# slowkow/scde

Hardware: AMD Instinct MI355X
Metric: genes/sec for scde.expression.difference (400-pt grid, 100 randomizations) (higher is better)
Workload: dtype f64; 1 GPU; config3: synthetic 20000 genes x 1000 cells (500/500), 401-pt grid, 100 bootstraps, n.cores=1 seeding; genes_total=20000, genes_per_gpu=20000, cells=1000, grid=401, n_randomizations=100, parallelism=gene-shard x1 (strong)

## Files before the change

### scde_amd/csrc/kernels.hip

```cpp
#include <hip/hip_runtime.h>
#include <algorithm>
#include <cmath>
#include <cstdint>
#include <utility>

#include "device_math.h"
#include "kernels.h"
#include "wave_ops.h"

namespace scde {

__global__ __launch_bounds__(256) void k_cell_prep(const double* __restrict__ models, int ncells, int G, int GS,
                                                   const double* __restrict__ mag, int localtheta,
                                                   int squarelogit, double* __restrict__ mu,
                                                   double* __restrict__ lcfp, double* __restrict__ lcfpr,
                                                   double* __restrict__ theta, double* __restrict__ cellscal,
                                                   double* __restrict__ pq, double* __restrict__ cfpo) {
  const int c = blockIdx.x;
  auto M = [&](int col) { return models[(long long)c + (long long)ncells * col]; };
  const double concb = M(0), conca = M(1), failr = M(2), corrb = M(3), corra = M(4), corrt = M(5);
  const double ltb = M(6), ltt = M(7), ltm = M(8), lts = M(9), ltr = M(10), conca2 = M(11);
  double lmax = -INFINITY;
  for (int k = threadIdx.x; k < G; k += blockDim.x) {
    const double m = mag[k];
// ... 307 lines not shown
  if (phase == 1) {
    c = blockIdx.x * 4 + wid;
    if (c >= a.ncells) return;
    const long long o1 = a.ucl_off[c + 1];
    long long zc = -1;
    for (long long i0 = a.ucl_off[c]; i0 < o1; i0 += 64) {
      const long long i = i0 + lane;
      const unsigned long long m = __ballot(i < o1 && a.ucl[i] == 0);
      if (m) {
        zc = i0 + __ffsll((long long)m) - 1;
        break;
      }
    }
    if (lane == 0) a.zcol[c] = zc >= 0 ? (int)zc + a.col_base : -1;
    if (zc < 0) {
      if (lane == 0) a.base_col[c] = -1;
      return;
    }
    col = zc;
  } else {
    col = (long long)blockIdx.x * 4 + wid;
    if (a.slow_only) {
      for (long long b0 = col * 64; b0 < a.ncols; b0 += (long long)gridDim.x * 4 * 64) {
        const long long ci = b0 + lane;
        unsigned long long m = __ballot(ci < a.ncols && !(a.colc[ci * kColc] > 0.0));
        while (m) {
          const long long cs = b0 + __ffsll((long long)m) - 1;
          m &= m - 1;
          int lo = 0, hi = a.ncells;
          while (hi - lo > 1) {
            const int mid = (lo + hi) >> 1;
            if (a.ucl_off[mid] <= cs) lo = mid; else hi = mid;
          }
          if (phase == 2 && cs == tab_zcol(a, lo)) continue;
          const long long co = (long long)lo * a.GS;
          const int bc = (phase == 2) ? tab_base_col(a, lo) : -1;
          const double* base = (bc >= 0 && a.D) ? a.D + (long long)bc * a.GS : nullptr;
          tables_column<CT>(a, cs, lo, phase, a.mu + co, (CT && a.pq) ? a.pq + 4 * co : nullptr, a.lcfpr + co,
                            a.lcfp + co, nullptr, nullptr, a.theta + co, base, vrow + (long long)wid * a.GS, etab,
                            lt, lane, a.GS);
        }
      }
      return;
    }
    if (phase == 2 && col == a.ncols) {
      for (int k = lane; k < a.GS; k += 64)
        if (a.D) a.D[col * a.GS + k] = 0.0;
      if (a.U && lane < kStretchSlots) a.U[col * kStretchSlots + lane] = 0.0;
      if (a.UQ && lane < kQTiles) a.UQ[col * kQTiles + lane] = 0u;
      return;
    }
    if (col >= a.ncols) return;
    int lo = 0, hi = a.ncells;
    while (hi - lo > 1) {
      const int mid = (lo + hi) >> 1;
      if (a.ucl_off[mid] <= col) lo = mid; else hi = mid;
    }
    c = lo;
    if (phase == 2 && col == tab_zcol(a, c)) return;
  }
  const long long co = (long long)c * a.GS;
  const int bc = (phase == 2) ? tab_base_col(a, c) : -1;
  const double* base = (bc >= 0 && a.D) ? a.D + (long long)bc * a.GS : nullptr;
  tables_column<CT>(a, col, c, phase, a.mu + co, (CT && a.pq) ? a.pq + 4 * co : nullptr, a.lcfpr + co,
                    a.lcfp + co, nullptr, nullptr, a.theta + co, base, vrow + (long long)wid * a.GS, etab, lt, lane,
                    a.GS);
}

constexpr int kTabStagedG = 448;
constexpr int kTabWaves = 8;
template <bool CT>
__global__ __launch_bounds__(64 * kTabWaves) __attribute__((amdgpu_waves_per_eu(SCDE_TAB_WPE))) void k_tables_cell(TablesArgs a) {
  extern __shared__ double dyn[];
  __shared__ double etab[64];
  __shared__ unsigned suqb[kQTiles];
  __shared__ double ltab[3][97];
  const int lane = threadIdx.x & 63, wid = threadIdx.x >> 6;
  const int GS = a.GS, G = a.G;
  tables_tabs(etab, ltab);
  if (a.gate && *a.gate == 0) return;
  const int4 task = a.tasks[blockIdx.x];
  const int c = task.x;
  const int phase = a.phase;
  if (c < 0) {
    if (wid == 0) {
      for (int k = lane; k < GS; k += 64)
        if (a.D) a.D[a.ncols * GS + k] = 0.0;
      if (a.U && lane < kStretchSlots) a.U[a.ncols * kStretchSlots + lane] = 0.0;
      if (a.UQ && lane < kQTiles) a.UQ[a.ncols * kQTiles + lane] = 0u;
    }
    return;
  }
  const bool haveP = CT && a.pq;
  double* smu = dyn + kTabWaves * G;
  double* sP = smu + G;
  double* slr = sP + 4 * G;
  double* slc = slr + G;
  double* sth = slc + G;
  double* sbase = sth + G;
  const long long co = (long long)c * GS;
  const int bc = (phase == 2) ? tab_base_col(a, c) : -1;
  if (bc >= 0 && a.UQ && threadIdx.x < kQTiles) suqb[threadIdx.x] = a.UQ[(long long)bc * kQTiles + threadIdx.x];
  for (int k = threadIdx.x; k < G; k += 64 * kTabWaves) {
    smu[k] = a.mu[co + k];
    slr[k] = a.lcfpr[co + k];
    slc[k] = exp(a.lcfp[co + k]);
    sth[k] = a.theta[co + k];
    if (haveP) {
      const double* P = a.pq + 4 * co;
      sP[k] = P[k];
      sP[G + k] = P[GS + k];
      sP[2 * G + k] = P[2 * GS + k];
      sP[3 * G + k] = P[3 * GS + k];
    }
    if (bc >= 0) sbase[k] = a.D[(long long)bc * GS + k];
  }
  __syncthreads();
  const LogTab lt{ltab[0], ltab[1], ltab[2]};
  const int zc = (phase == 2) ? tab_zcol(a, c) : -1;
  for (int col = task.y + wid; col < task.z; col += kTabWaves) {
    if (col == zc) continue;
    tables_column<CT>(a, col, c, phase, smu, haveP ? sP : nullptr, slr, nullptr, slc, (bc >= 0) ? suqb : nullptr, sth,
                      (bc >= 0) ? sbase : nullptr, dyn + wid * G, etab, lt, lane, G);
  }
}

constexpr int kTabChunks = kTabStagedG / 64;

constexpr int kRS = kTabStagedG;
enum { kRowMu = 0, kRowLP = 1, kRowLQ = 2, kRowLcfpr = 3, kRowCfp = 4, kRowLcfp = 5, kRowBase = 6, kTabRegRows = 7 };

enum { kBoundNone = 0, kBoundTiles = 1, kBoundStretch = 2 };
__device__ __forceinline__ void tab_store(double* p, double v, int nt) {
  if (nt)
    __builtin_nontemporal_store(v, p);
  else
    *p = v;
}
typedef double tab_v2d __attribute__((ext_vector_type(2)));
__device__ __forceinline__ void tab_store2(double* p, double a, double b, int nt) {
  tab_v2d v;
  v.x = a;
  v.y = b;
  if (nt)
    __builtin_nontemporal_store(v, reinterpret_cast<tab_v2d*>(p));
  else
    *reinterpret_cast<tab_v2d*>(p) = v;
}

template <int BM, int GC>
__device__ __forceinline__ void tables_column_reg(const TablesArgs& a, long long col, int c, int phase,
                                                  const double* __restrict__ sm, bool have_base,
                                                  const unsigned* __restrict__ uqb, const double* etab,
                                                  const LogTab& lt, int lane, double theta, const double* cc,
                                                  double x, double maxcfp, int bc_u) {
  const int G = GC ? GC : a.G;
  if (!(cc[0] > 0.0)) return;
  const double fp = cc[7];
  const double lpo = cc[8], lqo = cc[9];
  const double po = theta / (theta + x);
  if (SCDE_KT_DIAG & 32) {
    if (po == 12345.0) a.has_clamp[col] = 1;
    return;
  }
  const double* sl = sm + lane;
  double v[kTabChunks];
  double lmax = -INFINITY;
#pragma unroll
  for (int j = 0; j < kTabChunks; ++j) {
    v[j] = -INFINITY;
    if (64 * j < G) {
      const int k = lane + 64 * j;
      const bool in = k < G;
      const bool last = (k == G - 1);
      double lpr = sl[kRowLP * kRS + 64 * j], lqr = sl[kRowLQ * kRS + 64 * j];
      const double muv = sl[kRowMu * kRS + 64 * j], mnext = sl[kRowMu * kRS + 64 * j + 1];
      const bool over = in && ((!last && x > muv && x < mnext) || (last && x > muv));
      if (__builtin_amdgcn_ballot_w64(over)) {
        lpr = over ? lpo : lpr;
        lqr = over ? lqo : lqr;
      }
      double nb = (x == 0.0) ? theta * lpr : fma(x, lqr, fma(theta, lpr, cc[10]));
      nb += sl[kRowLcfpr * kRS + 64 * j];
      v[j] = in ? nb : -INFINITY;
      lmax = gt_max(lmax, v[j]);
    }
  }
  if (SCDE_KT_DIAG & 16) {
    if (lmax == 12345.0) a.has_clamp[col] = 1;
    return;
  }
  double maxp = wave_allreduce<true>(lmax);
  if (maxp < (maxcfp + fp)) maxp = maxcfp + fp;
  const double d0 = fp - maxp;
  const double E = exp_tab(fmax(d0, -746.0), etab);
  double ls = 0.0;
#pragma unroll
  for (int j = 0; j < kTabChunks; ++j) {
    if (64 * j < G) {
      const int k = lane + 64 * j;
      const bool in = k < G;
      v[j] -= maxp;
      double e = sl[kRowCfp * kRS + 64 * j] * E;
      if (!(SCDE_KT_DIAG & 2) && __builtin_amdgcn_ballot_w64(in && v[j] > -60.0)) e += exp_tab(fmax(v[j], -746.0), etab);
      ls += in ? e : 0.0;
    }
  }
  const double s = wave_allreduce<false>(ls);
  const double lsum = log_tab(s, lt);
  const bool want_maxi = a.maxi != nullptr;
  double bv = -INFINITY;
  int bi = 0x7fffffff;
  bool clamp = false, nanq = false;
  double* out = a.T ? a.T + col * a.GS : nullptr;
  double* dout = (phase && a.D) ? a.D + col * a.GS : nullptr;
  const double minlp = a.minlogprob;
  unsigned uqv = 0;
#pragma unroll
  for (int j = 0; j < kTabChunks; ++j) {
    if (64 * j < G) {
      const int k = lane + 64 * j;
      const bool in = k < G;
      const double t1 = v[j], t2 = sl[kRowLcfp * kRS + 64 * j] + d0;
      const double hi = gt_max(t2, t1), lo = (t1 > t2) ? t2 : t1;
      const bool tiny = !(hi >= -665.0);
      const bool mixed = !tiny && !(hi - lo > 37.5);
      double r = hi - lsum;
      if (__builtin_amdgcn_ballot_w64(in && (tiny || mixed))) {
        double e = fma(sl[kRowCfp * kRS + 64 * j], E, exp_tab(fmax(t1, -746.0), etab));
        if (__builtin_amdgcn_ballot_w64(in && tiny)) {
          const double et = exp_tab(fmax((sl[kRowLcfp * kRS + 64 * j] + fp) - maxp, -746.0), etab) +
                            exp_tab(fmax(t1, -746.0), etab);
          e = tiny ? et : e;
        }
        const double rm = (SCDE_KT_DIAG & 4) ? e - lsum : log_tab(tiny ? e / s : e, lt) - (tiny ? 0.0 : lsum);
        r = (tiny || mixed) ? rm : r;
      }
      if (want_maxi && r > bv && in) {
        bv = r;
        bi = k;
      }
      const bool cl = r < minlp;
      r = cl ? minlp : r;
      clamp = clamp || (cl && in);
      nanq = nanq || (in && r != r);
      if (!(SCDE_KT_DIAG & 8)) {
        if (out) tab_store(out + k, in ? r : 0.0, a.nt_rows);
        if (dout) tab_store(dout + k, in ? (have_base ? r - sl[kRowBase * kRS + 64 * j] : r) : 0.0, a.nt_rows);
      } else if (r == 12345.0) {
        dout[k] = r;
      }
      r = in ? r : -INFINITY;
      if (BM == kBoundTiles && !(SCDE_KT_DIAG & 64)) {
        int u = row16_max_i32((int)ceil(fmax(r * 256.0, -0x1p29)));
        const auto sw = __builtin_amdgcn_permlane16_swap((unsigned)u, (unsigned)u, false, false);
        u = max((int)sw[0], (int)sw[1]);
        const int g = __builtin_amdgcn_ds_bpermute(((lane - 2 * j) & 1) << 7, u);
        uqv = ((lane >> 1) == j) ? (unsigned)g : uqv;
      }
      if (BM == kBoundStretch) {
        const float mf = wave_maxf((float)r);
        if (lane == 0) {
          const double m = (double)mf + 0x1p-23 * fabs((double)mf);
          a.U[col * kStretchSlots + j] = (bc_u >= 0) ? m - a.U[(long long)bc_u * kStretchSlots + j] : m;
        }
      }
    }
  }
  if (BM == kBoundTiles) {
    if (__ballot(nanq) && lane == 0) *a.nanflag = 1;
    if (lane < kQTiles) {
      int u = (int)uqv;
      if (kBTile * lane >= G)
        u = 0;
      else if (bc_u >= 0)
        u -= unpacku(uqb[lane]);
      a.UQ[col * kQTiles + lane] = packu(u);
    }
  }
  if (dout)
    for (int k = 64 * ((G + 63) / 64) + lane; k < a.GS; k += 64) dout[k] = 0.0;
  if (want_maxi) {
#pragma unroll
    for (int m = 32; m >= 1; m >>= 1) {
      const double ov = __shfl_xor(bv, m, 64);
      const int oi = __shfl_xor(bi, m, 64);
      if (ov > bv || (ov == bv && oi < bi)) {
        bv = ov;
        bi = oi;
      }
    }
    if (lane == 0) a.maxi[col] = (bi == 0x7fffffff) ? 0 : bi;
  }
  const unsigned long long anyc = __ballot(clamp);
  if (lane == 0) a.has_clamp[col] = anyc ? 1 : 0;
}

#ifndef SCDE_LPC_DIAG
#define SCDE_LPC_DIAG 0
#endif
#ifndef LPC_U12
#define LPC_U12 4
#endif
#ifndef LPC_U3
#define LPC_U3 8
#endif
constexpr int kLpcWaves = 4;
constexpr int kLpcFlush = 8;
constexpr int kLpcTS = kLpcFlush + 1;
constexpr int kLpcQB = 0;
constexpr int kLpcLC = 2 * kTabStagedG;
constexpr int kLpcBase = 4 * kTabStagedG;
constexpr int kLpcR = 5 * kTabStagedG;
constexpr int kLpcMu = kLpcR;
constexpr int kLpcPart = kLpcR + kTabStagedG;
constexpr int kLpcRsz = kLpcWaves * 64 * kLpcTS;
constexpr int kLpcLds0 = kLpcR + kLpcRsz;
constexpr int kLpcLds = kLpcLds0 > kTabRegRows * kRS ? kLpcLds0 : kTabRegRows * kRS;
static_assert(kLpcRsz >= kTabStagedG + kLpcWaves * 64, "mu and the partials fit region R");
static_assert(kLpcWaves * 64 * 3 <= kLpcBase, "the combine's arrays overlay the staged rows");
static_assert(kTabTaskCols <= 64, "k_tables_lpc maps one lane to each column of a task: wider tasks would lose columns");

template <int BM>
__global__ __launch_bounds__(64 * kLpcWaves) void k_tables_lpc(TablesArgs a) {
  __shared__ __attribute__((aligned(16))) double lds[kLpcLds];
  __shared__ double etab[64];
  __shared__ unsigned suqb[kQTiles];
  __shared__ unsigned spart2[kLpcWaves][2][64];
  double(*spart)[64] = reinterpret_cast<double(*)[64]>(lds + kLpcPart);
  __shared__ int sfb[64];
  __shared__ int nfb;
  const int lane = threadIdx.x & 63;
  const int w = __builtin_amdgcn_readfirstlane(threadIdx.x >> 6);
  const int GS = a.GS, G = a.G;
  if (threadIdx.x < 64) etab[threadIdx.x] = kExp2Frac64[threadIdx.x];
  if (a.gate && *a.gate == 0) return;
  const int4 task = a.tasks[blockIdx.x];
  const int c = task.x;
  if (c < 0) {
    if (w == 0) {
      for (int k = lane; k < GS; k += 64)
        if (a.D) a.D[a.ncols * GS + k] = 0.0;
      if (a.U && lane < kStretchSlots) a.U[a.ncols * kStretchSlots + lane] = 0.0;
      if (a.UQ && lane < kQTiles) a.UQ[a.ncols * kQTiles + lane] = 0u;
    }
    return;
  }
  const int phase = a.phase;
  const long long co = (long long)c * GS;
  const int bc = (phase == 2) ? tab_base_col(a, c) : -1;
  if (bc >= 0 && a.UQ && threadIdx.x < kQTiles) suqb[threadIdx.x] = a.UQ[(long long)bc * kQTiles + threadIdx.x];
  if (threadIdx.x == 0) nfb = 0;
  const double theta = a.theta[co];
  const double* P = a.pq + 4 * co;
  int lean = theta > 0.0 && theta <= DBL_MAX;
  for (int k = threadIdx.x; k < kTabStagedG; k += 64 * kLpcWaves) {
    const bool in = k < G;
    double lq = 0.0, B = 0.0, lc = -INFINITY, cf = 0.0, base = 0.0, mu = 0.0;
    if (in) {
      mu = a.mu[co + k];
      const double lp = P[2 * GS + k], lr = a.lcfpr[co + k];
      lq = P[3 * GS + k];
      lc = a.lcfp[co + k];
      cf = a.cfp ? a.cfp[co + k] : exp(lc);
      B = fma(theta, lp, lr);
      if (bc >= 0) base = a.D[(long long)bc * GS + k];
      const bool ok = (k == G - 1 || mu <= a.mu[co + k + 1]) && lp <= DBL_MAX && lq <= DBL_MAX && lr <= DBL_MAX &&
                      lc <= DBL_MAX && cf <= DBL_MAX && cf == cf;
      lean &= ok ? 1 : 0;
    }
    lds[kLpcQB + 2 * k] = lq;
    lds[kLpcQB + 2 * k + 1] = B;
    lds[kLpcLC + 2 * k] = lc;
    lds[kLpcLC + 2 * k + 1] = cf;
    lds[kLpcBase + k] = base;
    lds[kLpcMu + k] = mu;
  }
  lean = __syncthreads_and(lean);
  const LogTab lt{kLogInvC, kLogCHi, kLogCLo};
  const int zc = (phase == 2) ? tab_zcol(a, c) : -1;
  const double maxcfp = a.cellscal[2 * c];
  const double minlp = a.minlogprob;
  const int col = task.y + lane;
  const bool mine = col < task.z && col != zc;
  double x = 1.0, c10 = 0.0, fp = 0.0, lpo = -1.0, lqo = -1.0;
  bool ok = false;
  if (mine) {
    const double* cc = a.colc + (long long)col * kColc;
    const double xx = (double)a.ucl[col], n = cc[0], cten = cc[10];
    if (lean && xx > 0.0 && n > 0.0 && cten >= -DBL_MAX && cten <= DBL_MAX) {
      ok = true;
      x = xx;
      c10 = cten;
      fp = cc[7];
      lpo = cc[8];
      lqo = cc[9];
    }
  }
  int ks = -1;
  double nb0o = 0.0;
  {
    int lo = 0, hi = G;
    while (lo < hi) {
      const int mid = (lo + hi) >> 1;
      if (lds[kLpcMu + mid] < x) lo = mid + 1; else hi = mid;
    }
    if (lo >= 1 && (lo == G || x < lds[kLpcMu + lo])) {
      ks = lo - 1;
      nb0o = fma(x, lqo, fma(theta, lpo, a.lcfpr[co + ks]));
    }
  }
  const int Gr = (G + kLpcFlush - 1) / kLpcFlush * kLpcFlush;
  const int per = max(64, (Gr / kLpcFlush + kLpcWaves - 1) / kLpcWaves * kLpcFlush);
  const int k0 = min(Gr, w * per), k1 = min(G, k0 + per), k1r = min(Gr, k0 + per);
  const double2* QB = reinterpret_cast<const double2*>(lds + kLpcQB);
  const double2* LC = reinterpret_cast<const double2*>(lds + kLpcLC);
  double m = -INFINITY;
#pragma unroll LPC_U12
  for (int k = k0; k < k1; ++k) {
    const double2 qb = QB[k];
    double nb = fma(x, qb.x, qb.y);
    nb = (k == ks) ? nb0o : nb;
    nb += c10;
    m = fmax(m, nb);
  }
  spart[w][lane] = m;
  __syncthreads();
  m = fmax(fmax(fmax(spart[0][lane], spart[1][lane]), spart[2][lane]), spart[3][lane]);
  double maxp = m;
  if (maxp < (maxcfp + fp)) maxp = maxcfp + fp;
  ok = ok && maxp > -INFINITY && maxp < INFINITY;
  if (!ok) maxp = 0.0;
  const double d0 = fp - maxp;
  const double E = exp_tab(fmax(d0, -746.0), etab);
  double ls = 0.0;
#pragma unroll LPC_U12
  for (int k = k0; k < k1; ++k) {
    const double2 qb = QB[k];
    const double cf = LC[k].y;
    const double t1 = (fma(x, qb.x, qb.y) + c10) - maxp;
    double e = cf * E;
    if (!(SCDE_LPC_DIAG & 2)) e += exp_tab(fmax(t1, -746.0), etab);
    ls += e;
  }
  if (ks >= k0 && ks < k1) {
    const double cf = LC[ks].y, tp = (fma(x, QB[ks].x, QB[ks].y) + c10) - maxp, to = (nb0o + c10) - maxp;
    ls += (cf * E + exp_tab(fmax(to, -746.0), etab)) - (cf * E + exp_tab(fmax(tp, -746.0), etab));
  }
  __syncthreads();
  spart[w][lane] = ls;
  __syncthreads();
  const double sq = ((spart[0][lane] + spart[1][lane]) + spart[2][lane]) + spart[3][lane];
  const double lsum = log_tab(sq, lt);
  __syncthreads();
  const bool want_maxi = a.maxi != nullptr;
  double bv = -INFINITY;
  int bi = 0x7fffffff;
  unsigned long long clampm = 0;
  const unsigned long long okm = __builtin_amdgcn_ballot_w64(ok);
  double* tw = lds + kLpcR + w * 64 * kLpcTS;
  double* const T = a.T;
  double* const D = (phase && a.D) ? a.D : nullptr;
  const long long cbase = task.y;
  constexpr int BSZ = (BM == kBoundStretch) ? 64 : kBTile;
  auto bound_form = [&](double mx) -> unsigned {
    if (BM == kBoundTiles) return (unsigned)(int)ceil(fmax(mx * 256.0, -0x1p29));
    return __float_as_uint((float)mx);
  };
  auto bound_max = [&](unsigned p, unsigned q) -> unsigned {
    if (BM == kBoundTiles) return (unsigned)max((int)p, (int)q);
    return __float_as_uint(fmaxf(__uint_as_float(p), __uint_as_float(q)));
  };
  auto put_bound = [&](int seg, unsigned form) {
    if (!ok) return;
    if (BM == kBoundTiles) {
      int u = (int)form;
      if (bc >= 0) u -= unpacku(suqb[seg]);
      a.UQ[(long long)col * kQTiles + seg] = packu(u);
    } else if (BM == kBoundStretch) {
      const float mf = __uint_as_float(form);
      const double mm = (double)mf + 0x1p-23 * fabs((double)mf);
      a.U[(long long)col * kStretchSlots + seg] = (bc >= 0) ? mm - a.U[(long long)bc * kStretchSlots + seg] : mm;
    }
  };
  double bt = -INFINITY;
  for (int f0 = k0; f0 < k1r; f0 += kLpcFlush) {
#pragma unroll LPC_U3
    for (int kk = 0; kk < kLpcFlush; ++kk) {
      const int k = f0 + kk;
      double r = 0.0;
      if (k < k1) {
        const double2 qb = QB[k], lcf = LC[k];
        double nb = fma(x, qb.x, qb.y);
        nb = (k == ks) ? nb0o : nb;
        const double t1 = (nb + c10) - maxp, t2 = lcf.x + d0;
        const double hi = fmax(t2, t1);
        const bool tiny = !(hi >= -665.0);
        const bool tm = tiny || !(fabs(t1 - t2) > 37.5);
        r = hi - lsum;
        if (!(SCDE_LPC_DIAG & 4) && __builtin_amdgcn_ballot_w64(ok && tm)) {
          double e = fma(lcf.y, E, exp_tab(fmax(t1, -746.0), etab));
          if (__builtin_amdgcn_ballot_w64(ok && tiny)) {
            const double et = exp_tab(fmax((lcf.x + fp) - maxp, -746.0), etab) + exp_tab(fmax(t1, -746.0), etab);
            e = tiny ? et / sq : e;
          }
          const double rm = log_tab(e, lt) - (tiny ? 0.0 : lsum);
          r = tm ? rm : r;
        }
        if (want_maxi) {
          const bool better = r > bv;
          bv = better ? r : bv;
          bi = better ? k : bi;
        }
        clampm |= __builtin_amdgcn_ballot_w64(r < minlp);
        r = fmax(r, minlp);
        if (BM != kBoundNone) {
          bt = fmax(bt, r);
          if ((k % BSZ) == BSZ - 1 || k == k1 - 1) {
            const int seg = k / BSZ;
            const bool head = seg * BSZ < k0, tail = (k % BSZ) != BSZ - 1 && k != G - 1;
            if (!head && !tail)
              put_bound(seg, bound_form(bt));
            else
              spart2[w][tail ? 1 : 0][lane] = bound_form(bt);
            bt = -INFINITY;
          }
        }
      }
      tw[lane * kLpcTS + kk] = r;
    }
#pragma unroll
    for (int i = 0; i < ((SCDE_LPC_DIAG & 1) ? 0 : 4); ++i) {
      const int cc_ = i * 16 + (lane >> 2), kp = (lane & 3) * 2;
      if ((okm >> cc_) & 1ull) {
        const double r0 = tw[cc_ * kLpcTS + kp], r1 = tw[cc_ * kLpcTS + kp + 1];
        const long long off = (cbase + cc_) * GS + f0 + kp;
        if (T) tab_store2(T + off, r0, r1, a.nt_rows);
        if (D) {
          const double2 bb = *reinterpret_cast<const double2*>(lds + kLpcBase + f0 + kp);
          tab_store2(D + off, r0 - bb.x, r1 - bb.y, a.nt_rows);
        }
      }
    }
  }
  const int GP = (SCDE_LPC_DIAG & 8) ? GS : min(GS, (G + 63) / 64 * 64);
  for (int f0 = Gr + kLpcFlush * w; f0 < GP; f0 += kLpcFlush * kLpcWaves) {
#pragma unroll
    for (int i = 0; i < 4; ++i) {
      const int cc_ = i * 16 + (lane >> 2), kp = (lane & 3) * 2;
      if ((okm >> cc_) & 1ull) {
        const long long off = (cbase + cc_) * GS + f0 + kp;
        const double z = ((SCDE_LPC_DIAG & 8) && f0 >= (G + 63) / 64 * 64) ? __builtin_nan("") : 0.0;
        if (T) tab_store2(T + off, z, z, a.nt_rows);
        if (D) tab_store2(D + off, z, z, a.nt_rows);
      }
    }
  }
  __syncthreads();
  double(*sclamp)[64] = reinterpret_cast<double(*)[64]>(lds);
  double(*sbv)[64] = reinterpret_cast<double(*)[64]>(lds + kLpcWaves * 64);
  int(*sbi)[64] = reinterpret_cast<int(*)[64]>(lds + 2 * kLpcWaves * 64);
  sclamp[w][lane] = ((clampm >> lane) & 1ull) ? 1.0 : 0.0;
  sbi[w][lane] = bi;
  sbv[w][lane] = bv;
  __syncthreads();
  if (w == 0 && ok) {
    a.has_clamp[col] = (sclamp[0][lane] + sclamp[1][lane] + sclamp[2][lane] + sclamp[3][lane] > 0.0) ? 1 : 0;
    if (want_maxi) {
      double b = sbv[0][lane];
      int bix = sbi[0][lane];
      for (int v = 1; v < kLpcWaves; ++v)
        if (sbv[v][lane] > b) {
          b = sbv[v][lane];
          bix = sbi[v][lane];
        }
      a.maxi[col] = (bix == 0x7fffffff) ? 0 : bix;
    }
  }
  if (BM != kBoundNone && w > 0 && (k0 % BSZ) != 0 && k0 < G)
    put_bound(k0 / BSZ, bound_max(spart2[w - 1][1][lane], spart2[w][0][lane]));
  if (BM == kBoundTiles && w == kLpcWaves - 1)
    for (int t = (G + kBTile - 1) / kBTile; t < kQTiles; ++t)
      if (ok) a.UQ[(long long)col * kQTiles + t] = packu(0);
  if (w == 0 && mine && !ok) sfb[atomicAdd(&nfb, 1)] = col;
  __syncthreads();
  const int nf = nfb;
  if (nf == 0) return;
  double* sm = lds;
  for (int k = threadIdx.x; k < kRS; k += 64 * kLpcWaves) {
    const bool in = k < G;
    sm[kRowMu * kRS + k] = in ? a.mu[co + k] : 0.0;
    sm[kRowLP * kRS + k] = in ? P[2 * GS + k] : 0.0;
    sm[kRowLQ * kRS + k] = in ? P[3 * GS + k] : 0.0;
    sm[kRowLcfpr * kRS + k] = in ? a.lcfpr[co + k] : 0.0;
    const double lc = in ? a.lcfp[co + k] : -INFINITY;
    sm[kRowCfp * kRS + k] = in ? (a.cfp ? a.cfp[co + k] : exp(lc)) : 0.0;
    sm[kRowLcfp * kRS + k] = lc;
    sm[kRowBase * kRS + k] = (in && bc >= 0) ? a.D[(long long)bc * GS + k] : 0.0;
  }
  __syncthreads();
  for (int i = w; i < nf; i += kLpcWaves) {
    const int fc = __builtin_amdgcn_readfirstlane(sfb[i]);
    tables_column_reg<BM, 0>(a, fc, c, phase, sm, bc >= 0, suqb, etab, lt, lane, theta, a.colc + (long long)fc * kColc,
                             (double)a.ucl[fc], maxcfp, bc);
  }
}

__global__ void k_base_cols(const int* __restrict__ ucl, const long long* __restrict__ ucl_off, int ncells,
                            const unsigned char* __restrict__ has_clamp, int use_baseline,
                            int* __restrict__ base_col) {
  const int c = blockIdx.x * blockDim.x + threadIdx.x;
  if (c >= ncells) return;
  int bc = -1;
  if (use_baseline) {
    for (long long i = ucl_off[c]; i < ucl_off[c + 1]; ++i) {
      if (ucl[i] == 0) {
        if (!has_clamp[i]) bc = (int)i;
        break;
      }
    }
  }
  base_col[c] = bc;
}

__global__ __launch_bounds__(256) void k_delta(const double* __restrict__ T, const long long* __restrict__ ucl_off,
                                              int ncells, long long ncols, const int* __restrict__ base_col, int G,
                                              int GS, double* __restrict__ D) {
  const int lane = threadIdx.x & 63;
  const long long col = (long long)blockIdx.x * 4 + (threadIdx.x >> 6);
  if (col > ncols) return;
  if (col == ncols) {
    for (int k = lane; k < GS; k += 64) D[col * GS + k] = 0.0;
    return;
  }
  int lo = 0, hi = ncells;
  while (hi - lo > 1) {
    const int mid = (lo + hi) >> 1;
    if (ucl_off[mid] <= col) lo = mid; else hi = mid;
  }
  const int bc = base_col[lo];
  for (int k = lane; k < GS; k += 64) {
    const double t = (k < G) ? T[col * GS + k] : 0.0;
    D[col * GS + k] = (bc >= 0 && k < G) ? t - T[(long long)bc * GS + k] : t;
  }
}

constexpr int kZWaves = 16;
__global__ __launch_bounds__(64 * kZWaves) void k_baseline_z(const double* __restrict__ T, int G, int GS,
                                                            const int* __restrict__ base_col, int ncells,
                                                            const double* __restrict__ Wt, int Bp,
                                                            double* __restrict__ Z, int gsets, int gsplit) {
  __shared__ double part[kZWaves][4][64];
  const int lane = threadIdx.x & 63, wid = threadIdx.x >> 6;
  const int b0 = blockIdx.x * 4, k = blockIdx.y * 64 + lane, set = blockIdx.z;
  const double* W = Wt + (long long)set * ncells * Bp + b0;
  const bool g2 = gsets > 0 && set >= gsets;
  const int clo = g2 ? gsplit : 0, chi = (gsets > 0 && !g2) ? gsplit : ncells;
  double z[4] = {0.0, 0.0, 0.0, 0.0};
  if (k < G) {
    for (int c = clo + wid; c < chi; c += kZWaves) {
      const int bc = base_col[c];
      if (bc < 0) continue;
      const double t = T[(long long)bc * GS + k];
      const double* w = W + (long long)c * Bp;
#pragma unroll
      for (int r = 0; r < 4; ++r) z[r] = fma(w[r], t, z[r]);
    }
  }
#pragma unroll
  for (int r = 0; r < 4; ++r) part[wid][r][lane] = z[r];
  __syncthreads();
  if (wid < 4 && k < GS) {
    double s = part[0][wid][lane];
#pragma unroll
    for (int w = 1; w < kZWaves; ++w) s += part[w][wid][lane];
    Z[((long long)set * Bp + b0 + wid) * GS + k] = s;
  }
}

__global__ __launch_bounds__(256) void k_stretch_zu(const double* __restrict__ U, const int* __restrict__ base_col,
                                                    int ncells, const double* __restrict__ Wt, int Bp,
                                                    double* __restrict__ ZU, int gsets, int gsplit) {
  __shared__ double part[256][kStretchSlots + 1];
  const int b = blockIdx.x, set = blockIdx.y, t = threadIdx.x;
  const double* W = Wt + (long long)set * ncells * Bp + b;
  const bool g2 = gsets > 0 && set >= gsets;
  const int clo = g2 ? gsplit : 0, chi = (gsets > 0 && !g2) ? gsplit : ncells;
  double z[kStretchSlots];
#pragma unroll
  for (int j = 0; j < kStretchSlots; ++j) z[j] = 0.0;
  for (int c = clo + t; c < chi; c += 256) {
    const int bc = base_col[c];
    if (bc < 0) continue;
    const double w = W[(long long)c * Bp];
    const double* u = U + (long long)bc * kStretchSlots;
#pragma unroll
    for (int j = 0; j < kStretchSlots; ++j) z[j] = fma(w, u[j], z[j]);
  }
#pragma unroll
  for (int j = 0; j < kStretchSlots; ++j) part[t][j] = z[j];
  __syncthreads();
  for (int h = 128; h >= 1; h >>= 1) {
    if (t < h)
#pragma unroll
      for (int j = 0; j < kStretchSlots; ++j) part[t][j] += part[t + h][j];
    __syncthreads();
  }
  if (t < kStretchSlots) ZU[((long long)set * Bp + b) * kStretchSlots + t] = part[0][t];
}

template <int BC, bool MAX>
__device__ __forceinline__ double wave_reduce_scatter_v(double (&v)[BC], int lane) {
  static_assert(BC == 4 || BC == 8 || BC == 16, "BC must be 4, 8 or 16");
#pragma unroll
  for (int j = 0; j < BC / 2; ++j) {
    swap32(v[j], v[j + BC / 2]);
    v[j] = red_op<MAX>(v[j], v[j + BC / 2]);
  }
#pragma unroll
  for (int j = 0; j < BC / 4; ++j) {
    swap16(v[j], v[j + BC / 4]);
    v[j] = red_op<MAX>(v[j], v[j + BC / 4]);
  }
  if constexpr (BC >= 8) {
    const bool up = (lane & 8) != 0;
#pragma unroll
    for (int j = 0; j < BC / 8; ++j) {
      const double lo = v[j], hi = v[j + BC / 8];
      v[j] = red_op<MAX>(up ? hi : lo, dpp_d<kDppMirror>(up ? lo : hi));
    }
  }
  if constexpr (BC >= 16) {
    const bool up = (lane & 4) != 0;
    const double lo = v[0], hi = v[1];
    v[0] = red_op<MAX>(up ? hi : lo, dpp_d<kDppHalfMirror>(up ? lo : hi));
  }
  double x = v[0];
  if constexpr (BC <= 4) x = red_op<MAX>(x, dpp_d<kDppMirror>(x));
  if constexpr (BC <= 8) x = red_op<MAX>(x, dpp_d<kDppHalfMirror>(x));
  x = red_op<MAX>(x, dpp_d<kDppXor2>(x));
  x = red_op<MAX>(x, dpp_d<kDppXor1>(x));
  return x;
}

template <int BC, bool MAX, int NB>
__device__ __forceinline__ void wave_partials(const double (&x)[NB], int I0, bool live, double* red, int lane,
                                              int wid) {
  constexpr int L2 = (BC == 16) ? 4 : (BC == 8) ? 3 : (BC == 4) ? 2 : (BC == 2) ? 1 : 0;
  double t[BC];
#pragma unroll
  for (int i = 0; i < BC; ++i) t[i] = x[I0 + i];
  const double r = wave_reduce_scatter_v<BC, MAX>(t, lane);
  const int idx = (lane >> (6 - L2)) & (BC - 1);
  if ((lane & ((64 >> L2) - 1)) == 0) red[wid * 32 + I0 + idx] = r;
}

template <bool MAX, int NB>
__device__ __forceinline__ void block_reduce_all(const double (&x)[NB], bool live, double* red, double* fin,
                                                 int lane, int wid, int nw) {
#pragma unroll
  for (int i0 = 0; i0 + 16 <= NB; i0 += 16) wave_partials<16, MAX, NB>(x, i0, live, red, lane, wid);
  if constexpr ((NB % 16) >= 8) wave_partials<8, MAX, NB>(x, NB - (NB % 16), live, red, lane, wid);
  if constexpr ((NB % 8) >= 4) wave_partials<4, MAX, NB>(x, NB - (NB % 8), live, red, lane, wid);
  __syncthreads();
  if ((int)threadIdx.x < NB) {
    double r = red[threadIdx.x];
    for (int w = 1; w < nw; ++w) r = MAX ? gt_max(r, red[w * 32 + threadIdx.x]) : r + red[w * 32 + threadIdx.x];
    fin[threadIdx.x] = r;
  }
  __syncthreads();
}


template <int BC>
__device__ __forceinline__ float wave_max_scatter_f(float (&v)[BC], int lane) {
  static_assert(BC == 4 || BC == 8 || BC == 16, "BC must be 4, 8 or 16");
#pragma unroll
  for (int j = 0; j < BC / 2; ++j) {
    swap32f(v[j], v[j + BC / 2]);
    v[j] = gt_maxf(v[j], v[j + BC / 2]);
  }
#pragma unroll
  for (int j = 0; j < BC / 4; ++j) {
    swap16f(v[j], v[j + BC / 4]);
    v[j] = gt_maxf(v[j], v[j + BC / 4]);
  }
  if constexpr (BC >= 8) {
    const bool up = (lane & 8) != 0;
#pragma unroll
    for (int j = 0; j < BC / 8; ++j) {
      const float lo = v[j], hi = v[j + BC / 8];
      v[j] = gt_maxf(up ? hi : lo, dpp_f<kDppMirror>(up ? lo : hi));
    }
  }
  if constexpr (BC >= 16) {
    const bool up = (lane & 4) != 0;
    const float lo = v[0], hi = v[1];
    v[0] = gt_maxf(up ? hi : lo, dpp_f<kDppHalfMirror>(up ? lo : hi));
  }
  float x = v[0];
  if constexpr (BC <= 4) x = gt_maxf(x, dpp_f<kDppMirror>(x));
  if constexpr (BC <= 8) x = gt_maxf(x, dpp_f<kDppHalfMirror>(x));
  x = gt_maxf(x, dpp_f<kDppXor2>(x));
  x = gt_maxf(x, dpp_f<kDppXor1>(x));
  return x;
}

template <int BC, int NB>
__device__ __forceinline__ void wave_max_partials(const double (&x)[NB], int I0, float* redf, int lane, int wid) {
  constexpr int L2 = (BC == 16) ? 4 : (BC == 8) ? 3 : 2;
  float t[BC];
// ... 1659 lines not shown
```

Baseline: 3.053 million genes/s.

## Compact divergent exp/log lanes into dense wave work lists per flush block

The flush loop now runs in two passes. The first pass computes a cheap approximation for each of the 8 grid points and records a per-lane bitmask of points that need the exact exp/log path. Lanes with any such point are compacted into a per-wave LDS list. The wave then processes 8 lanes x 8 points per iteration, fetching each source lane's parameters with shuffles, so the expensive transcendental path runs with dense lanes instead of mostly idle divergent ones. The exact results go through the tw scratch buffer, which adds LDS traffic, shuffles and a serial loop over the list; this could cost more than it saves when few lanes diverge or when nearly all do.

```diff
diff --git a/scde_amd/csrc/kernels.hip b/scde_amd/csrc/kernels.hip
--- a/scde_amd/csrc/kernels.hip
+++ b/scde_amd/csrc/kernels.hip
@@ -633,9 +633,6 @@
 #ifndef LPC_U12
 #define LPC_U12 4
 #endif
-#ifndef LPC_U3
-#define LPC_U3 8
-#endif
 constexpr int kLpcWaves = 4;
 constexpr int kLpcFlush = 8;
 constexpr int kLpcTS = kLpcFlush + 1;
@@ -661,6 +658,7 @@
   double(*spart)[64] = reinterpret_cast<double(*)[64]>(lds + kLpcPart);
   __shared__ int sfb[64];
   __shared__ int nfb;
+  __shared__ unsigned short slist[kLpcWaves][64];
   const int lane = threadIdx.x & 63;
   const int w = __builtin_amdgcn_readfirstlane(threadIdx.x >> 6);
   const int GS = a.GS, G = a.G;
@@ -815,29 +813,65 @@
     }
   };
   double bt = -INFINITY;
+  unsigned short* const wl = slist[w];
   for (int f0 = k0; f0 < k1r; f0 += kLpcFlush) {
-#pragma unroll LPC_U3
+    double rr[kLpcFlush];
+    unsigned fm = 0;
+#pragma unroll
     for (int kk = 0; kk < kLpcFlush; ++kk) {
       const int k = f0 + kk;
-      double r = 0.0;
+      rr[kk] = 0.0;
       if (k < k1) {
         const double2 qb = QB[k], lcf = LC[k];
         double nb = fma(x, qb.x, qb.y);
         nb = (k == ks) ? nb0o : nb;
         const double t1 = (nb + c10) - maxp, t2 = lcf.x + d0;
         const double hi = fmax(t2, t1);
+        const bool tm = !(hi >= -665.0) || !(fabs(t1 - t2) > 37.5);
+        rr[kk] = hi - lsum;
+        fm |= (ok && tm) ? (1u << kk) : 0u;
+      }
+    }
+    if (!(SCDE_LPC_DIAG & 4) && __builtin_amdgcn_ballot_w64(fm != 0)) {
+      const unsigned long long bal = __builtin_amdgcn_ballot_w64(fm != 0);
+      const int nl = __popcll(bal);
+      if (fm) wl[__builtin_amdgcn_mbcnt_hi((unsigned)(bal >> 32), __builtin_amdgcn_mbcnt_lo((unsigned)bal, 0u))] =
+          (unsigned short)(lane | (fm << 6));
+#pragma unroll 1
+      for (int r0 = 0; r0 < nl; r0 += 8) {
+        const int j = r0 + (lane >> 3);
+        const int ent = j < nl ? (int)wl[j] : lane;
+        const int sl = ent & 63, kp = lane & 7, k = f0 + kp;
+        const bool live = (ent >> (6 + kp)) & 1;
+        const double xs = __shfl(x, sl, 64), c10s = __shfl(c10, sl, 64), maxps = __shfl(maxp, sl, 64);
+        const double fps = __shfl(fp, sl, 64), Es = __shfl(E, sl, 64), lsums = __shfl(lsum, sl, 64);
+        const double nb0s = __shfl(nb0o, sl, 64);
+        const int kss = __shfl(ks, sl, 64);
+        const double2 qb = QB[k], lcf = LC[k];
+        double nb = fma(xs, qb.x, qb.y);
+        nb = (k == kss) ? nb0s : nb;
+        const double d0s = fps - maxps;
+        const double t1 = (nb + c10s) - maxps, t2 = lcf.x + d0s;
+        const double hi = fmax(t2, t1);
         const bool tiny = !(hi >= -665.0);
-        const bool tm = tiny || !(fabs(t1 - t2) > 37.5);
-        r = hi - lsum;
-        if (!(SCDE_LPC_DIAG & 4) && __builtin_amdgcn_ballot_w64(ok && tm)) {
-          double e = fma(lcf.y, E, exp_tab(fmax(t1, -746.0), etab));
-          if (__builtin_amdgcn_ballot_w64(ok && tiny)) {
-            const double et = exp_tab(fmax((lcf.x + fp) - maxp, -746.0), etab) + exp_tab(fmax(t1, -746.0), etab);
-            e = tiny ? et / sq : e;
-          }
-          const double rm = log_tab(e, lt) - (tiny ? 0.0 : lsum);
-          r = tm ? rm : r;
+        double e = fma(lcf.y, Es, exp_tab(fmax(t1, -746.0), etab));
+        if (__builtin_amdgcn_ballot_w64(live && tiny)) {
+          const double sqs = __shfl(sq, sl, 64);
+          const double et = exp_tab(fmax((lcf.x + fps) - maxps, -746.0), etab) + exp_tab(fmax(t1, -746.0), etab);
+          e = tiny ? et / sqs : e;
         }
+        const double rm = log_tab(e, lt) - (tiny ? 0.0 : lsums);
+        if (live) tw[sl * kLpcTS + kp] = rm;
+      }
+#pragma unroll
+      for (int kk = 0; kk < kLpcFlush; ++kk)
+        if ((fm >> kk) & 1u) rr[kk] = tw[lane * kLpcTS + kk];
+    }
+#pragma unroll
+    for (int kk = 0; kk < kLpcFlush; ++kk) {
+      const int k = f0 + kk;
+      double r = rr[kk];
+      if (k < k1) {
         if (want_maxi) {
           const bool better = r > bv;
           bv = better ? r : bv;
```

New measurement: 2.985 million genes/s. -2.2%, worse.
